# reglab/aquaculture

Measured on AMD Instinct MI355X. Metric: 640px tiles/sec (whole node) YOLOv5m bf16, higher is better.
Workload: dtype bf16

## Files before the change

aquaculture_amd/csrc/detect_nms.hip:

```cpp
#include "aq_common.h"

namespace {

constexpr float kMaxWH = 7680.0f;
constexpr int kMaxNms = 30000;
constexpr int kNmsThreads = 1024;
constexpr int kSortLds = 4096;

struct DecodeParams {
    const float* head[3];
    int head_ld;
    int B, nc, na, no;
    int ny[3], nx[3];
    int off[4];
    float stride[3];
    float anchor[3][8][2];
    float* pred;
    float conf_thres;
    int32_t* cand;
    float* cand_rows;
    int32_t* cand_count;
    int cap;
    int lmask, base, pred_rows;
    float scale, flip_w;
// ... 82 lines not shown
                if (p.cand_rows)
                    decode_row<AUG>(p, src[k], lvl[k], a[k], x[k], y[k], obj[k], p.cand_rows + ((long long)b * p.cap + pos) * p.no);
            }
        }
    }
}

struct NmsParams {
    const float* rows;
    int rows_per_tile;
    int B, N, nc, no;
    float conf_thres, iou_thres;
    int max_det;
    const int32_t* cand;
    const int32_t* cand_count;
    int cap;
    unsigned long long* keys;
    float4* sbox;
    unsigned long long* mask;
    int npow2;
    aq_det* dets;
    int32_t* counts;
    unsigned long long* dbg;
    float class_step;
    unsigned long long cls_lo, cls_hi;
};

constexpr int kFast = 2048;
constexpr int kFastBig = 4096;
constexpr int kFastRowsLimit = 40000;
__host__ __device__ constexpr int nms_fast(int N) { return N > kFastRowsLimit ? kFastBig : kFast; }
constexpr int kIdxBits = 17;
constexpr int nms_fast_lds(int kf) { return kf * 8 + kf * 16 + kf * 4 + kf * 2; }
constexpr int nms_mask_lds(int kf) { return kf == kFast ? 64 * 1024 : 32 * 1024; }
constexpr int kSlowLds = kSortLds * 8 + kMaxNms + 16;
constexpr int nms_lds(int kf) { return nms_fast_lds(kf) + nms_mask_lds(kf) > kSlowLds ? nms_fast_lds(kf) + nms_mask_lds(kf) : kSlowLds; }
static_assert(nms_lds(kFastBig) <= 160 * 1024, "LDS");

__device__ __forceinline__ bool candidate_row(const float* row, int nc, float thr, float4& box, float& conf, int& cls,
                                              unsigned long long cls_lo = ~0ULL, unsigned long long cls_hi = ~0ULL) {
    const float obj = row[4];
    if (!(obj > thr)) return false;
    float best = row[5] * obj;
    int bj = 0;
    for (int c = 1; c < nc; ++c) {
        const float v = row[5 + c] * obj;
        if (v > best) { best = v; bj = c; }
    }
    if (!(best > thr)) return false;
// ... 43 lines not shown
    if (!(inter > 0.0f)) return false;
    const float jarea = (bj.z - bj.x) * (bj.w - bj.y);
    const float uni = iarea + jarea - inter;
    const float q = inter * __builtin_amdgcn_rcpf(uni);
    if (q > thr_hi) return true;
    if (q < thr_lo) return false;
    return inter / uni > thr;
}

__device__ __forceinline__ unsigned long long readlane64(unsigned long long v, int lane) {
    const unsigned lo = (unsigned)__builtin_amdgcn_readlane((int)(unsigned)(v & 0xffffffffull), lane);
    const unsigned hi = (unsigned)__builtin_amdgcn_readlane((int)(unsigned)(v >> 32), lane);
    return ((unsigned long long)hi << 32) | lo;
}

template <int KF>
__global__ __launch_bounds__(kNmsThreads) void nms_kernel(const NmsParams p) {
    constexpr int kFast = KF, kFastWords = KF / 64, kFastLds = nms_fast_lds(KF), kMaskLds = nms_mask_lds(KF);
    __shared__ int s_n;
    extern __shared__ __attribute__((aligned(16))) unsigned char s_raw[];
    __shared__ int s_kept;
    const int b = blockIdx.x, tid = threadIdx.x;
    auto stamp = [&](int i) { if (p.dbg && tid == 0) p.dbg[(long long)b * 8 + i] = clock64(); };
    stamp(0);
    const float* rows = p.rows + (long long)b * p.rows_per_tile * p.no;
    unsigned long long* keys = p.keys + (long long)b * p.npow2;

    if (tid == 0) s_n = 0;
    __syncthreads();
    const int n0 = p.cand ? min(p.cand_count[b], p.cap) : p.N;
    for (int t = tid; t < n0; t += kNmsThreads) {
        const int idx = p.cand ? p.cand[(long long)b * p.cap + t] : t;
        float4 box; float conf; int cls;
        if (candidate_row(rows + (long long)t * p.no, p.nc, p.conf_thres, box, conf, cls, p.cls_lo, p.cls_hi)) {
            const int pos = atomicAdd(&s_n, 1);
            keys[pos] = make_key(conf, idx, t);
        }
    }
    __syncthreads();
    stamp(1);
    int n = s_n;
    if (n == 0) {
        if (tid == 0) p.counts[b] = 0;
        return;
    }

    auto emit = [&](int slot, int k) {
        float4 box; float conf; int cls;
        candidate_row(rows + (long long)slot * p.no, p.nc, p.conf_thres, box, conf, cls, p.cls_lo, p.cls_hi);
        aq_det d; d.x1 = box.x; d.y1 = box.y; d.x2 = box.z; d.y2 = box.w; d.conf = conf; d.cls = (float)cls;
        p.dets[(long long)b * p.max_det + k] = d;
    };

    if (n <= kFast) {
        unsigned long long* kin = (unsigned long long*)s_raw;
        float4* sb = (float4*)(s_raw + kFast * 8);
        int* sslot = (int*)(s_raw + kFast * 8 + kFast * 16);
        unsigned short* skept = (unsigned short*)(s_raw + kFast * 8 + kFast * 16 + kFast * 4);
        for (int t = tid; t < n; t += kNmsThreads) kin[t] = keys[t];
        __syncthreads();
        for (int t = tid; t < n; t += kNmsThreads) {
            const unsigned long long k = kin[t];
            int r = 0;
            for (int u = 0; u < n; ++u) r += (kin[u] > k) ? 1 : 0;
            sslot[r] = key_slot(k);
            float4 box; float conf; int cls;
            candidate_row(rows + (long long)key_slot(k) * p.no, p.nc, p.conf_thres, box, conf, cls, p.cls_lo, p.cls_hi);
            const float c = (float)cls * p.class_step;
            box.x = box.x + c; box.y = box.y + c; box.z = box.z + c; box.w = box.w + c;
            sb[r] = box;
        }
        __syncthreads();
        stamp(2);
        const int nw = (n + 63) >> 6;
        const float thr_lo = p.iou_thres * (1.0f - 4e-7f), thr_hi = p.iou_thres * (1.0f + 4e-7f);
        auto matrix_and_scan = [&](unsigned long long* mask) __attribute__((always_inline)) {
            int total_items = 0;
            for (int bi = 0; bi < nw; ++bi) total_items += 64 * (nw - bi);
            for (int item = tid; item < total_items; item += kNmsThreads) {
                int bi = 0, rem = item;
                while (rem >= 64 * (nw - bi)) { rem -= 64 * (nw - bi); ++bi; }
                const int wpr = nw - bi;
                const int i = 64 * bi + rem / wpr, w = bi + rem % wpr;
                if (i >= n) continue;
                const float4 bi4 = sb[i];
                const float iarea = (bi4.z - bi4.x) * (bi4.w - bi4.y);
                const int j0 = w << 6;
                const int jbeg = max(j0, i + 1), jend = min(j0 + 64, n);
                unsigned long long bits = 0ull;
#pragma unroll 4
                for (int j = jbeg; j < jend; ++j)
                    if (iou_gt_fast(bi4, iarea, sb[j], p.iou_thres, thr_lo, thr_hi)) bits |= 1ull << (j - j0);
                mask[(long long)i * nw + w] = bits;
            }
            __syncthreads();
            stamp(3);
            if (tid < 64) {
                unsigned long long removed = 0ull;
                int kept = 0;
                bool done = false;
                for (int w = 0; w < nw && !done; ++w) {
                    const int i_l = 64 * w + tid;
                    const unsigned long long diag = i_l < n ? mask[(long long)i_l * nw + w] : 0ull;
                    const int left = n - 64 * w;
                    const unsigned long long valid = left >= 64 ? ~0ull : ((1ull << left) - 1ull);
                    unsigned long long alive = valid & ~readlane64(removed, w);
                    unsigned long long keptmask = 0ull;
                    while (alive != 0ull) {
                        const int bit = __builtin_ctzll(alive);
                        keptmask |= 1ull << bit;
                        alive &= ~(1ull << bit);
                        alive &= ~readlane64(diag, bit);
                        if (kept + __builtin_popcountll(keptmask) >= p.max_det) { done = true; break; }
                    }
                    if ((keptmask >> tid) & 1ull)
                        skept[kept + __builtin_popcountll(keptmask & ((1ull << tid) - 1ull))] = (unsigned short)(64 * w + tid);
                    kept += __builtin_popcountll(keptmask);
                    unsigned long long km = keptmask, acc = 0ull;
                    const bool mine = tid > w && tid < nw;
                    while (km != 0ull) {
                        int bits4[4];
#pragma unroll
                        for (int u = 0; u < 4; ++u) {
                            bits4[u] = km != 0ull ? __builtin_ctzll(km) : -1;
                            km &= km - 1ull;
                        }
                        unsigned long long r4[4];
#pragma unroll
                        for (int u = 0; u < 4; ++u) r4[u] = (mine && bits4[u] >= 0) ? mask[(long long)(64 * w + bits4[u]) * nw + tid] : 0ull;
                        acc |= (r4[0] | r4[1]) | (r4[2] | r4[3]);
                    }
                    removed |= acc;
                }
                if (tid == 0) { p.counts[b] = kept; s_kept = kept; }
            }
        };
        if ((size_t)n * nw * 8 <= kMaskLds) matrix_and_scan((unsigned long long*)(s_raw + kFastLds));
        else matrix_and_scan(p.mask + (long long)b * kFast * kFastWords);
        __syncthreads();
        stamp(4);
        for (int k = tid; k < s_kept; k += kNmsThreads) emit(sslot[skept[k]], k);
        __syncthreads();
        stamp(5);
        return;
    }

    unsigned long long* s_keys = (unsigned long long*)s_raw;
    unsigned char* s_supp = s_raw + kSortLds * 8;
// ... 110 lines not shown
    return align_up((size_t)B * next_pow2(N) * sizeof(unsigned long long), 256) + align_up((size_t)B * N * sizeof(float4), 256) +
           align_up((size_t)B * nms_fast(N) * (nms_fast(N) / 64) * sizeof(unsigned long long), 256);
}

extern "C" int aq_nms(const float* rows_dev, int rows_per_tile, int B, int N, int nc, float conf_thres, float iou_thres,
                      int max_det, const int32_t* cand_dev, const int32_t* cand_count_dev, int cand_cap,
                      void* scratch_dev, aq_det* dets_dev, int32_t* counts_dev, void* stream) {
    return aq_nms_opts(rows_dev, rows_per_tile, B, N, nc, conf_thres, iou_thres, max_det, cand_dev, cand_count_dev, cand_cap, scratch_dev, dets_dev,
                       counts_dev, 0, ~0ULL, ~0ULL, stream);
}

extern "C" int aq_nms_opts(const float* rows_dev, int rows_per_tile, int B, int N, int nc, float conf_thres, float iou_thres,
                           int max_det, const int32_t* cand_dev, const int32_t* cand_count_dev, int cand_cap,
                           void* scratch_dev, aq_det* dets_dev, int32_t* counts_dev, int agnostic, unsigned long long classes_lo,
                           unsigned long long classes_hi, void* stream) {
    AQ_REQUIRE(nc <= 128, "nms: the class filter covers 128 classes (nc = %d)", nc);
    AQ_REQUIRE(rows_dev && scratch_dev && dets_dev && counts_dev, "nms: null pointer");
    AQ_REQUIRE(B > 0 && N > 0 && nc >= 1 && max_det > 0, "nms: bad shape B=%d N=%d nc=%d max_det=%d", B, N, nc, max_det);
    AQ_REQUIRE(N < (1 << kIdxBits), "nms: at most %d candidates per tile are supported (got %d)", (1 << kIdxBits) - 1, N);
    AQ_REQUIRE(!cand_dev || (cand_count_dev && cand_cap > 0 && cand_cap <= N && rows_per_tile == cand_cap),
               "nms: a compact candidate list needs a counter, 0 < cap <= N and rows_per_tile == cap");
    AQ_REQUIRE(cand_dev || rows_per_tile == N, "nms: without a candidate list the rows are the full pred (rows_per_tile == N)");
    NmsParams p;
    p.rows = rows_dev; p.rows_per_tile = rows_per_tile; p.B = B; p.N = N; p.nc = nc; p.no = nc + 5;
    p.conf_thres = conf_thres; p.iou_thres = iou_thres; p.max_det = max_det;
    p.cand = cand_dev; p.cand_count = cand_count_dev; p.cap = cand_cap;
    p.class_step = agnostic ? 0.0f : kMaxWH; p.cls_lo = classes_lo; p.cls_hi = classes_hi;
    p.npow2 = next_pow2(N);
    char* s = (char*)scratch_dev;
    p.keys = (unsigned long long*)s;
    s += align_up((size_t)B * p.npow2 * sizeof(unsigned long long), 256);
    p.sbox = (float4*)s;
    s += align_up((size_t)B * N * sizeof(float4), 256);
    p.mask = (unsigned long long*)s;
    p.dets = dets_dev; p.counts = counts_dev;
    p.dbg = aq_stamp_target((size_t)B * 64);
    const bool big = nms_fast(N) == kFastBig;
    auto fn = big ? nms_kernel<kFastBig> : nms_kernel<kFast>;
    const int lds = nms_lds(big ? kFastBig : kFast);
    AQ_CHECK_HIP(aq_kernel_lds((const void*)fn, lds));
    hipLaunchKernelGGL(fn, dim3(B), dim3(kNmsThreads), lds, (hipStream_t)stream, p);
// ... 4 lines not shown
```

aquaculture_amd/csrc/engine.cpp:

```cpp
#include "aq_common.h"
#include <unistd.h>
#include <string>

#include <cstdarg>
#include <cstdio>
#include <cstdlib>
#include <cstring>
#include <string>
#include <atomic>
#include <dlfcn.h>
#include <vector>

namespace {
thread_local char g_err[512] = "";
}

void aq_set_error(const char* fmt, ...) {
    va_list ap;
    va_start(ap, fmt);
    vsnprintf(g_err, sizeof(g_err), fmt, ap);
    va_end(ap);
}

extern "C" const char* aq_last_error(void) { return g_err; }
// ... 134 lines not shown
    struct Tuned { int B = 0, H = 0, W = 0; std::vector<int> cfg; };
    std::vector<Tuned> tuned;
    int tuned_cur = -1;
    bool tuning = false;
    void* zero_page = nullptr;
    int lay_B = 0, lay_H = 0, lay_W = 0;
    bool lay_aug = false;
    int run_H = 0, run_W = 0;
    std::vector<TensorPlace> place;
    size_t off_pred = 0, off_cand = 0, off_cand_rows = 0, off_cand_count = 0, off_cand_wide = 0, off_nms = 0, off_taps = 0, total_bytes = 0;
    int N = 0;
    aq_augment_pass aug[3] = {};
    std::vector<int> aug_family[3], aug_cfg[3];
    void* last_ws = nullptr;
    const uint8_t* last_tiles = nullptr;
    float* calib_amax = nullptr;
    std::vector<int> last_family, last_cfg;
    bool prof = false;
    int ring = 0;
    long long prof_calls = 0;
    std::vector<hipEvent_t> ev;
};

namespace {

void set_dims(aq_engine* e, int H, int W) {
    for (size_t t = 0; t < e->tensors.size(); ++t) {
        e->place[t].h = H / e->tensors[t].down;
        e->place[t].w = W / e->tensors[t].down;
    }
// ... 396 lines not shown
                float anchors[8 * 2];
                for (int a = 0; a < e->desc.na; ++a) {
                    anchors[2 * a] = e->desc.anchors_px[op.level][a][0];
                    anchors[2 * a + 1] = e->desc.anchors_px[op.level][a][1];
                }
                note_launch(e, oi, AQ_FAM_HEAD_DECODE);
                if (ar) {
                    rc = aq_head_decode_aug(tptr(e, ws, tiles, op.src.tensor), e->tensors[op.src.tensor].channels, op.src.ch_off, op.src.channels,
                                            e->packed[oi].w_head, B, pl.h, pl.w, aug_base + off, e->desc.stride[op.level], anchors, e->desc.nc, e->desc.na,
                                            conf, aug_scale, aug_flip_w, cand, cand_rows, wide, kCountStride, e->N, stream);
                    break;
                }
                rc = aq_head_decode(tptr(e, ws, tiles, op.src.tensor), e->tensors[op.src.tensor].channels, op.src.ch_off, op.src.channels,
                                    e->packed[oi].w_head, B, pl.h, pl.w, off, e->desc.stride[op.level], anchors, e->desc.nc, e->desc.na, conf,
                                    cand, cand_rows, wide, kCountStride, e->N, stream);
                if (!rc && ++heads_done == 3) rc = aq_head_counts_gather(wide, kCountStride, cand_count, B, stream);
                break;
            }
            rc = run_conv(e, oi, ws, tiles, B, stream);
            if (!rc && e->calib_amax && e->tensors[op.dst.tensor].dtype == AQ_T_ACT && prec == AQ_BF16 && op.dst.channels % 8 == 0) {
                const TensorPlace& pdc = e->place[op.dst.tensor];
                rc = aq_absmax_bf16(tptr(e, ws, tiles, op.dst.tensor), e->tensors[op.dst.tensor].channels, op.dst.ch_off, op.dst.channels,
                                    (long long)B * pdc.h * pdc.w, e->calib_amax + oi, stream);
            }
            break;
        case AQ_OP_STEM:
            note_launch(e, oi, AQ_FAM_STEM);
            if (stemdown) break;
            if (scaled) {
                rc = aq_stem_conv_scaled(tiles, ar->H0, ar->W0, ar->ytab, ar->xtab, ar->ps->h, ar->ps->w, tptr(e, ws, tiles, op.dst.tensor),
                                         e->tensors[op.dst.tensor].channels, op.dst.ch_off, op.dst.channels, e->packed[oi].w, e->packed[oi].bias,
// ... 38 lines not shown
        case AQ_OP_SPPF_POOL: {
            const TensorPlace& pl = e->place[op.src.tensor];
            rc = aq_sppf_pool(tptr(e, ws, tiles, op.src.tensor), e->tensors[op.src.tensor].channels, op.src.ch_off,
                              op.src.channels, B, pl.h, pl.w, prec, stream);
            break;
        }
        case AQ_OP_UPSAMPLE2X: {
            const TensorPlace& pl = e->place[op.src.tensor];
            rc = aq_upsample2x(tptr(e, ws, tiles, op.src.tensor), e->tensors[op.src.tensor].channels, op.src.ch_off,
                               tptr(e, ws, tiles, op.dst.tensor), e->tensors[op.dst.tensor].channels, op.dst.ch_off,
                               op.src.channels, B, pl.h, pl.w, prec, stream);
            break;
        }
        case AQ_OP_DECODE: {
            if (fuse_heads) break;
            const float* heads[3];
            for (int l = 0; l < 3; ++l) heads[l] = (const float*)tptr(e, ws, tiles, e->desc.head_tensor[l]);
            float anchors[3 * 8 * 2];
            for (int l = 0; l < 3; ++l)
                for (int a = 0; a < e->desc.na; ++a) {
                    anchors[(l * e->desc.na + a) * 2] = e->desc.anchors_px[l][a][0];
                    anchors[(l * e->desc.na + a) * 2 + 1] = e->desc.anchors_px[l][a][1];
                }
            const bool want_nms = dets != nullptr;
            if (ar) {
                rc = aq_detect_decode_aug(heads, e->tensors[e->desc.head_tensor[0]].channels, B, H, W, e->desc.nc, e->desc.na, anchors,
                                          e->desc.stride, ar->ps->level_mask, aug_base, e->N, aug_scale, aug_flip_w, want_nms ? nullptr : pred,
                                          conf, want_nms ? cand : nullptr, want_nms ? cand_rows : nullptr, want_nms ? cand_count : nullptr,
                                          e->N, stream);
                break;
            }
            rc = aq_detect_decode(heads, e->tensors[e->desc.head_tensor[0]].channels, B, H, W, e->desc.nc, e->desc.na,
                                  anchors, e->desc.stride, want_nms ? nullptr : pred, conf, want_nms ? cand : nullptr,
                                  want_nms ? cand_rows : nullptr, want_nms ? cand_count : nullptr, e->N, stream);
            break;
        }
        case AQ_OP_NMS:
            if (dets && !ar)
                rc = aq_nms_opts(cand_rows, e->N, B, e->N, e->desc.nc, conf, iou, max_det, cand, cand_count, e->N,
                                 (char*)ws + e->off_nms, dets, counts, e->nms_agnostic, e->nms_cls_lo, e->nms_cls_hi, stream);
            break;
        default:
            aq_set_error("unknown op kind %d", op.kind);
            rc = AQ_ERR_INVALID;
        }
        if (mark) g_roctx.pop();
        if (rc) return rc;
    }
    if (ev) {
        AQ_CHECK_HIP(hipEventRecord(ev[n_ops], stream));
        e->prof_calls++;
    }
    return AQ_OK;
}

// ... 28 lines not shown
    if (dets) {
        AQ_CHECK_HIP(hipMemsetAsync(fuse ? wide : cand_count, 0, sizeof(int32_t) * B * (fuse ? kCountStride : 1), stream));
    }
    float* pred = pred_out ? pred_out : (float*)((char*)ws + e->off_pred);
    for (int i = 0; i < 3 && !rc; ++i) {
        const aq_augment_pass& ps = e->aug[i];
        const AugRun ar{i, &ps, H, W, ytab[i], xtab[i]};
        set_dims(e, ps.hp, ps.wp);
        if (e->last_family.size() == e->ops.size()) { e->last_family.assign(e->ops.size(), AQ_FAM_NONE); e->last_cfg.assign(e->ops.size(), -1); }
        rc = run_plan(e, tiles, B, ps.hp, ps.wp, ws, ws_bytes, pred, dets, counts, conf, iou, max_det, stream, 0, -1, &ar);
        e->aug_family[i] = e->last_family;
        e->aug_cfg[i] = e->last_cfg;
    }
    set_dims(e, H, W);
    if (rc || !dets) return rc;
    if (fuse) {
        rc = aq_head_counts_gather(wide, kCountStride, cand_count, B, stream);
        if (rc) return rc;
    }
    return aq_nms_opts((float*)((char*)ws + e->off_cand_rows), e->N, B, e->N, e->desc.nc, conf, iou, max_det, (int32_t*)((char*)ws + e->off_cand),
                       cand_count, e->N, (char*)ws + e->off_nms, dets, counts, e->nms_agnostic, e->nms_cls_lo, e->nms_cls_hi, stream);
}

}

extern "C" int aq_pack_conv_weights(const float* w, int cout, int k, int cin, int precision, void* packed_dev,
                                    size_t* bytes, void* stream) {
    AQ_REQUIRE(w && bytes, "pack: null pointer");
    AQ_REQUIRE(cout > 0 && k > 0 && cin > 0 && (cin * aq_elem_bytes(precision)) % 16 == 0,
               "pack: cin=%d must make whole 16-byte groups", cin);
    std::vector<unsigned char> host;
    int kg, kgp, g, rows;
    pack_host(w, cout, k, cin, precision, host, &kg, &kgp, &g, &rows);
    *bytes = host.size();
    if (packed_dev) {
        AQ_CHECK_HIP(hipMemcpyAsync(packed_dev, host.data(), host.size(), hipMemcpyHostToDevice, (hipStream_t)stream));
// ... 101 lines not shown
    if (x3) compute_desc.precision = AQ_FP32;
    d = &compute_desc;
    e->desc = *d;
    e->tensors.assign(d->tensors, d->tensors + d->n_tensors);
    e->ops.assign(d->ops, d->ops + d->n_ops);
    e->desc.tensors = e->tensors.data();
    e->desc.ops = e->ops.data();
    e->packed.resize(e->ops.size());
    e->conv_cfg.assign(e->ops.size(), -1);
    const int eb = aq_elem_bytes(d->precision);
    auto fail = [&](int rc) { aq_engine_destroy(e); return rc; };
    if (hipMalloc(&e->zero_page, 4096) != hipSuccess || hipMemset(e->zero_page, 0, 4096) != hipSuccess) {
        aq_set_error("engine_create: zero page allocation failed");
        return fail(AQ_ERR_NOMEM);
    }
    const char* use_tail = getenv("AQ_C3TAIL");
    for (size_t oi = 0; d->precision == AQ_BF16 && !(use_tail && *use_tail == '0') && oi + 1 < e->ops.size(); ++oi) {
        const aq_op_desc& b = e->ops[oi];
        const aq_op_desc& c = e->ops[oi + 1];
        if (b.kind != AQ_OP_BOTTLENECK || c.kind != AQ_OP_CONV || !b.weight || !b.bias || !c.weight || !c.bias) continue;
        if (b.src.channels != 48 || b.dst.channels != 48 || b.k != 3 || b.dst.tensor < 0 || b.dst.tensor >= d->n_tensors || b.dst.ch_off != 0 ||
            e->tensors[b.dst.tensor].channels != 96 || b.src.tensor == b.dst.tensor)
            continue;
        if (c.k != 1 || c.stride != 1 || c.act != 1 || c.res.tensor >= 0 || c.level >= 0 || c.src.tensor != b.dst.tensor || c.src.ch_off != 0 ||
            c.src.channels != 96 || c.dst.channels != 96 || c.dst.tensor < 0 || c.dst.tensor >= d->n_tensors || c.dst.tensor == c.src.tensor ||
            c.dst.tensor == b.src.tensor || c.dst.ch_off % 8 || e->tensors[c.dst.tensor].channels % 8 || e->tensors[c.dst.tensor].dtype != AQ_T_ACT)
            continue;
        bool read_later = false;
        for (size_t oj = oi + 2; oj < e->ops.size(); ++oj)
            for (const aq_slice* s : {&e->ops[oj].src, &e->ops[oj].res})
// ... 353 lines not shown

extern "C" int aq_engine_tensor_ptr(aq_engine* e, int tensor, void** ptr, int* channels, int* h, int* w, int* elem_bytes) {
    AQ_REQUIRE(e && ptr && tensor >= 0 && tensor < (int)e->tensors.size(), "tensor_ptr: bad tensor id %d", tensor);
    AQ_REQUIRE(e->last_ws, "tensor_ptr: no call has run yet");
    *ptr = tptr(e, e->last_ws, e->last_tiles, tensor);
    if (channels) *channels = e->tensors[tensor].channels;
    if (h) *h = e->place[tensor].h;
    if (w) *w = e->place[tensor].w;
    if (elem_bytes) *elem_bytes = e->place[tensor].elem;
    return AQ_OK;
}

extern "C" int aq_engine_candidates(aq_engine* e, void** cand, void** rows, void** counts, int* cap) {
    AQ_REQUIRE(e && cand && rows && counts && cap, "candidates: null pointer");
    AQ_REQUIRE(e->last_ws, "candidates: no call has run yet");
    *cand = (char*)e->last_ws + e->off_cand;
    *rows = (char*)e->last_ws + e->off_cand_rows;
    *counts = (char*)e->last_ws + e->off_cand_count;
    *cap = e->N;
    return AQ_OK;
}

extern "C" int aq_engine_num_ops(aq_engine* e) { return e ? (int)e->ops.size() : 0; }

extern "C" int aq_engine_set_nms_options(aq_engine* e, int agnostic, unsigned long long classes_lo, unsigned long long classes_hi) {
    AQ_REQUIRE(e, "set_nms_options: null engine");
    e->nms_agnostic = agnostic != 0; e->nms_cls_lo = classes_lo; e->nms_cls_hi = classes_hi;
    return AQ_OK;
}

// ... 168 lines not shown
```

aquaculture_amd/engine.py:

```python
from __future__ import annotations

import ctypes as C
import os
import re
from typing import Dict, List, Optional, Sequence, Tuple

import numpy as np
import torch

from . import spec as _spec
from .checkpoint import Checkpoint, pack_plan_weights

AQ_BF16, AQ_FP32, AQ_BF16_W8, AQ_F16X3 = 0, 1, 2, 3
PRECISIONS = {"bf16": AQ_BF16, "fp32": AQ_FP32, "fp8w": AQ_BF16, "f16x3": AQ_F16X3}
"""Compute precision of the single-op helpers.  fp8w = fp8 (OCP e4m3fn) weights with per-output-channel power-of-two scales, bf16
activations (quant.py): values bf16 holds exactly, so every bf16 kernel runs them as they are."""
ENGINE_PRECISIONS = {"bf16": AQ_BF16, "fp32": AQ_FP32, "fp8w": AQ_BF16_W8, "f16x3": AQ_F16X3, "fp8": AQ_BF16}
"""aq_model_desc.precision.  AQ_BF16_W8 computes as AQ_BF16; kernels with an fp8-weight stream (the planar 3x3) load the e4m3 codes."""
_DTYPE_CODE = {"act": 0, "f32": 1, "u8": 2}

LIB_PATH = os.path.join(os.path.dirname(os.path.abspath(__file__)), "csrc", "libaqengine.so")


class aq_tensor_desc(C.Structure):
# ... 17 lines not shown
                ("head_tensor", C.c_int32 * 3), ("input_tensor", C.c_int32),
                ("n_tensors", C.c_int32), ("n_ops", C.c_int32),
                ("tensors", C.POINTER(aq_tensor_desc)), ("ops", C.POINTER(aq_op_desc))]


class aq_det(C.Structure):
    _fields_ = [("x1", C.c_float), ("y1", C.c_float), ("x2", C.c_float), ("y2", C.c_float),
                ("conf", C.c_float), ("cls", C.c_float)]


EXPORTS = (
    "aq_last_error", "aq_version", "aq_engine_create", "aq_engine_destroy", "aq_engine_workspace_bytes", "aq_size_guard",
    "aq_engine_infer", "aq_engine_run_ops", "aq_engine_candidates", "aq_engine_forward_raw", "aq_engine_tensor_ptr", "aq_engine_profile",
    "aq_engine_op_times", "aq_engine_num_ops", "aq_engine_set_conv_config", "aq_engine_autotune", "aq_engine_set_tuned_table",
    "aq_engine_get_conv_config", "aq_conv_num_configs", "aq_debug_conv_stamp", "aq_debug_mfma_peak",
    "aq_conv_config_tiles", "aq_pack_conv_weights", "aq_pack_conv_weights_x3", "aq_conv2d", "aq_pack_stem_weights", "aq_stem_conv", "aq_pack_bottleneck_weights", "aq_bottleneck", "aq_bottleneck_asm_form", "aq_bottleneck_c3tail_supported", "aq_pack_bottleneck_c3tail_weights", "aq_bottleneck_c3tail", "aq_pack_downblock_weights", "aq_downblock", "aq_stemdown_supported", "aq_stemdown", "aq_conv1x1_direct_supported", "aq_pack_conv1x1_direct", "aq_conv1x1_direct", "aq_conv1x1_asm_supported", "aq_pack_conv1x1_asm", "aq_conv1x1_asm", "aq_nms_opts", "aq_engine_set_nms_options",
    "aq_conv3x3s2_direct_supported", "aq_pack_conv3x3s2_direct", "aq_conv3x3s2_direct",
    "aq_conv3x3_pl_supported", "aq_conv3x3_pl_asm_family", "aq_pack_conv3x3_pl", "aq_conv3x3_pl", "aq_conv3x3_pl_s2_supported", "aq_pack_conv3x3_pl_s2", "aq_conv3x3_pl_s2", "aq_jpeg_scratch_bytes", "aq_jpeg_idct_rgb", "aq_jpeg_idct_rgb_checked", "aq_f32_to_e4m3", "aq_conv1x1_direct_f8out", "aq_absmax_bf16", "aq_engine_calibrate_amax", "aq_engine_set_fp8_scales", "aq_engine_last_launch", "aq_conv3x3_pl_f8_supported", "aq_pack_conv3x3_pl_f8", "aq_conv3x3_pl_f8", "aq_conv3x3_pl_w8_supported", "aq_pack_conv3x3_pl_w8", "aq_conv3x3_pl_w8", "aq_head_decode_supported", "aq_pack_head_weights", "aq_head_decode", "aq_head_counts_gather", "aq_preprocess_s2d", "aq_sppf_pool",
    "aq_upsample2x", "aq_letterbox_u8", "aq_letterbox_tiles_u8", "aq_format_label_rows", "aq_detect_decode", "aq_nms_scratch_bytes", "aq_nms", "aq_jpeg_huffman_decode", "aq_write_label_files",
    "aq_crop_jpeg_coefs", "aq_crop_jpeg_bytes", "aq_write_crop_files",
    "aq_annotate_u8", "aq_image_jpeg_coefs", "aq_image_jpeg_bytes", "aq_write_image_files",
    "aq_blank_stats_scratch_bytes", "aq_blank_stats_u8",
    "aq_blank_geom_scratch_bytes", "aq_blank_components_u8", "aq_blank_ring_edges_u8",
    "aq_facility_scratch_bytes", "aq_facility_dbscan_f64",
    "aq_land_scratch_bytes", "aq_land_filter_f64",
    "aq_eval_scratch_bytes", "aq_eval_member_conf_f64", "aq_box_match_f64",
    "aq_eval_subsets_scratch_bytes", "aq_eval_member_conf_subsets_f64", "aq_box_match_subsets_scratch_bytes", "aq_box_match_subsets_f64",
    "aq_model_error_match_f64", "aq_model_error_moments_f64",
    "aq_tonnage_simulate_f64", "aq_tonnage_reduce_f64", "aq_tonnage_ndtri_f64", "aq_tonnage_uniform_f64",
    "aq_depth_ranges_f64", "aq_depth_stats_f64",
    "aq_dedup_fill_u32", "aq_dedup_sets_u32", "aq_dedup_select_f64",
# ... 93 lines not shown
                              i32, i32, i32, i32, i32, i32, i32, i32, i32, vp, vp]
    lib.aq_pack_stem_weights.argtypes = [C.POINTER(f32), i32, i32, vp, C.POINTER(sz), vp]
    lib.aq_stem_conv.argtypes = [vp, vp, i32, i32, i32, vp, vp, i32, i32, i32, i32, i32, vp]
    lib.aq_pack_bottleneck_weights.argtypes = [C.POINTER(f32), C.POINTER(f32), i32, vp, C.POINTER(sz), vp]
    lib.aq_bottleneck.argtypes = [vp, i32, i32, vp, i32, i32, i32, vp, vp, i32, i32, i32, i32, vp]
    lib.aq_bottleneck_asm_form.argtypes = [i32] * 6
    lib.aq_bottleneck_c3tail_supported.argtypes = [i32, i32, i32, i32, i32, i32]
    lib.aq_pack_bottleneck_c3tail_weights.argtypes = [C.POINTER(f32), C.POINTER(f32), C.POINTER(f32), vp, C.POINTER(sz), vp]
    lib.aq_bottleneck_c3tail.argtypes = [vp, i32, i32, vp, i32, i32, vp, i32, i32, vp, vp, i32, i32, i32, i32, vp]
    lib.aq_pack_downblock_weights.argtypes = [C.POINTER(f32), C.POINTER(f32), vp, C.POINTER(sz), vp]
    lib.aq_downblock.argtypes = [vp, i32, i32, vp, i32, i32, vp, vp, i32, i32, i32, vp]
    lib.aq_conv1x1_direct_supported.argtypes = [i32, i32]
    lib.aq_pack_conv1x1_direct.argtypes = [C.POINTER(f32), i32, i32, vp, C.POINTER(sz), vp]
    lib.aq_conv1x1_direct.argtypes = [vp, i32, i32, vp, i32, i32, i32, i32, vp, vp, C.c_longlong, i32, vp]
    lib.aq_nms_opts.argtypes = [vp, i32, i32, i32, i32, f32, f32, i32, vp, vp, i32, vp, vp, vp, i32, C.c_ulonglong, C.c_ulonglong, vp]
    lib.aq_engine_set_nms_options.argtypes = [vp, i32, C.c_ulonglong, C.c_ulonglong]
    lib.aq_conv1x1_asm_supported.argtypes = [i32, i32]
    lib.aq_pack_conv1x1_asm.argtypes = [C.POINTER(f32), i32, i32, vp, C.POINTER(sz), vp]
    lib.aq_conv1x1_asm.argtypes = [vp, i32, i32, vp, i32, i32, i32, i32, vp, vp, C.c_longlong, i32, vp]
    lib.aq_conv3x3s2_direct_supported.argtypes = [i32, i32]
    lib.aq_pack_conv3x3s2_direct.argtypes = [C.POINTER(f32), i32, i32, vp, C.POINTER(sz), vp]
    lib.aq_conv3x3s2_direct.argtypes = [vp, i32, i32, vp, i32, i32, i32, i32, vp, vp, i32, i32, i32, i32, vp]
    lib.aq_conv3x3_pl_supported.argtypes = [i32, i32]
    lib.aq_conv3x3_pl_asm_family.argtypes = [i32]
    lib.aq_pack_conv3x3_pl.argtypes = [C.POINTER(f32), i32, i32, vp, C.POINTER(sz), vp]
    lib.aq_conv3x3_pl.argtypes = [vp, C.c_longlong, C.c_longlong, i32, vp, i32, i32, i32, vp, i32, i32, vp, vp, i32, i32, i32, i32, vp]
    lib.aq_conv3x3_pl_w8.argtypes = lib.aq_conv3x3_pl.argtypes
    lib.aq_pack_conv3x3_pl_w8.argtypes = [C.POINTER(C.c_float), C.POINTER(C.c_float), i32, i32, vp, C.POINTER(C.c_size_t), vp, vp]
    lib.aq_conv3x3_pl_w8_supported.argtypes = [i32] * 5
    lib.aq_jpeg_scratch_bytes.argtypes = [i32, i32, i32]
# ... 380 lines not shown
    lib = load_library()
    if pred.dtype != torch.float32 or pred.dim() != 3 or not pred.is_cuda or not pred.is_contiguous():
        raise ValueError("pred must be a contiguous CUDA float32 tensor [B, N, 5+nc]")
    B, N, no = pred.shape
    if no != nc + 5:
        raise ValueError(f"pred last dim {no} != nc + 5 = {nc + 5}")
    scratch = torch.empty(lib.aq_nms_scratch_bytes(B, N), dtype=torch.uint8, device=pred.device)
    dets = torch.empty((B, max_det, 6), dtype=torch.float32, device=pred.device)
    counts = torch.empty((B,), dtype=torch.int32, device=pred.device)
    lo, hi = class_mask(classes, nc)
    _check(lib.aq_nms_opts(pred.data_ptr(), N, B, N, nc, conf_thres, iou_thres, max_det, None, None, 0,
                           scratch.data_ptr(), dets.data_ptr(), counts.data_ptr(), int(bool(agnostic)), lo, hi, _stream_ptr()))
    return dets, counts


_zero_pages: Dict[int, torch.Tensor] = {}


def _zero_page(device) -> torch.Tensor:
    key = device.index or 0
    if key not in _zero_pages:
        _zero_pages[key] = torch.zeros(4096, dtype=torch.uint8, device=device)
    return _zero_pages[key]


def pack_conv_weights(w_oihw: torch.Tensor, precision: str, device) -> torch.Tensor:
    lib = load_library()
    prec = PRECISIONS[precision]
    w = np.ascontiguousarray(w_oihw.permute(0, 2, 3, 1).float().cpu().numpy())
    cout, k, _, cin = w.shape
# ... 1540 lines not shown
```

include/aq_engine.h:

```cpp
#ifndef AQ_ENGINE_H
#define AQ_ENGINE_H

#include <stddef.h>
#include <stdint.h>

#ifdef __cplusplus
extern "C" {
#endif

typedef enum aq_status {
    AQ_OK = 0,
    AQ_ERR_INVALID = -1,
    AQ_ERR_HIP = -2,
    AQ_ERR_NOMEM = -3,
    AQ_ERR_WORKSPACE = -4
} aq_status;

typedef enum aq_precision {
    AQ_BF16 = 0,
    AQ_FP32 = 1,
    AQ_BF16_W8 = 2,
    AQ_F16X3 = 3
} aq_precision;

// ... 215 lines not shown
                   int32_t* cand_dev, float* cand_rows_dev, int32_t* cand_count_dev, int count_stride, int cand_cap, void* stream);
int aq_head_counts_gather(const int32_t* wide_dev, int count_stride, int32_t* compact_dev, int B, void* stream);

int aq_detect_decode(const float* const head_dev[3], int head_ld, int B, int H, int W, int nc, int na,
                     const float* anchors_px , const float* stride ,
                     float* pred_dev, float conf_thres, int32_t* cand_dev, float* cand_rows_dev,
                     int32_t* cand_count_dev, int cand_cap, void* stream);
size_t aq_nms_scratch_bytes(int B, int N);
int aq_nms(const float* rows_dev, int rows_per_tile, int B, int N, int nc, float conf_thres, float iou_thres,
           int max_det, const int32_t* cand_dev, const int32_t* cand_count_dev, int cand_cap,
           void* scratch_dev, aq_det* dets_dev, int32_t* counts_dev, void* stream);
int aq_nms_opts(const float* rows_dev, int rows_per_tile, int B, int N, int nc, float conf_thres, float iou_thres,
                int max_det, const int32_t* cand_dev, const int32_t* cand_count_dev, int cand_cap,
                void* scratch_dev, aq_det* dets_dev, int32_t* counts_dev, int agnostic, unsigned long long classes_lo,
                unsigned long long classes_hi, void* stream);
int aq_engine_set_nms_options(aq_engine* e, int agnostic, unsigned long long classes_lo, unsigned long long classes_hi);

typedef struct aq_augment_pass {
    float scale;
    int32_t flip;
    int32_t h, w;
    int32_t hp, wp;
    int32_t rows;
    int32_t keep_first, keep_count;
    int32_t out_first;
    int32_t level_mask;
} aq_augment_pass;
int aq_augment_geometry(int H, int W, int na, aq_augment_pass passes_out[3], int* n_aug);
typedef struct aq_tap { int32_t i0, i1; float l0, l1; } aq_tap;
int aq_augment_taps(int in, int out, int flip, aq_tap* taps_host);
// ... 129 lines not shown
```

Baseline: 17210.

## Split NMS into per-class segments and read strided candidate counters directly

When NMS is class-aware, candidates are bucketed by class into contiguous segments. Each class then gets its own triangular IoU mask and greedy scan, run in parallel across waves, instead of one n-by-n matrix scanned by a single wave. Kept boxes are compacted back into score order with a prefix scan. Separately, the NMS kernel now reads the wide per-tile counters through a stride, which removes the counts-gather launch on the default path. The cost is extra sorting and class-rank work, more LDS bookkeeping, and a fallback whenever box coordinates exceed the segment bound.

```diff
diff --git a/aquaculture_amd/csrc/detect_nms.hip b/aquaculture_amd/csrc/detect_nms.hip
--- a/aquaculture_amd/csrc/detect_nms.hip
+++ b/aquaculture_amd/csrc/detect_nms.hip
@@ -120,7 +120,9 @@
     int max_det;
     const int32_t* cand;
     const int32_t* cand_count;
+    int count_stride;
     int cap;
+    int segments;
     unsigned long long* keys;
     float4* sbox;
     unsigned long long* mask;
@@ -139,6 +141,8 @@
 constexpr int kIdxBits = 17;
 constexpr int nms_fast_lds(int kf) { return kf * 8 + kf * 16 + kf * 4 + kf * 2; }
 constexpr int nms_mask_lds(int kf) { return kf == kFast ? 64 * 1024 : 32 * 1024; }
+constexpr int kSegTab = 4096;
+constexpr float kSegCoord = 3712.0f;
 constexpr int kSlowLds = kSortLds * 8 + kMaxNms + 16;
 constexpr int nms_lds(int kf) { return nms_fast_lds(kf) + nms_mask_lds(kf) > kSlowLds ? nms_fast_lds(kf) + nms_mask_lds(kf) : kSlowLds; }
 static_assert(nms_lds(kFastBig) <= 160 * 1024, "LDS");
@@ -212,10 +216,63 @@
     return ((unsigned long long)hi << 32) | lo;
 }
 
+__device__ __forceinline__ void matrix_word(const float4* sb, int n, int nw, int i, int w, float thr, float thr_lo, float thr_hi,
+                                            unsigned long long* mask) {
+    const float4 bi4 = sb[i];
+    const float iarea = (bi4.z - bi4.x) * (bi4.w - bi4.y);
+    const int j0 = w << 6;
+    const int jbeg = max(j0, i + 1), jend = min(j0 + 64, n);
+    unsigned long long bits = 0ull;
+#pragma unroll 4
+    for (int j = jbeg; j < jend; ++j)
+        if (iou_gt_fast(bi4, iarea, sb[j], thr, thr_lo, thr_hi)) bits |= 1ull << (j - j0);
+    mask[(long long)i * nw + w] = bits;
+}
+
+template <class Kept>
+__device__ __forceinline__ int greedy_scan(const unsigned long long* mask, int n, int nw, int lane, int max_det, Kept&& on_kept) {
+    unsigned long long removed = 0ull;
+    int kept = 0;
+    bool done = false;
+    for (int w = 0; w < nw && !done; ++w) {
+        const int i_l = 64 * w + lane;
+        const unsigned long long diag = i_l < n ? mask[(long long)i_l * nw + w] : 0ull;
+        const int left = n - 64 * w;
+        const unsigned long long valid = left >= 64 ? ~0ull : ((1ull << left) - 1ull);
+        unsigned long long alive = valid & ~readlane64(removed, w);
+        unsigned long long keptmask = 0ull;
+        while (alive != 0ull) {
+            const int bit = __builtin_ctzll(alive);
+            keptmask |= 1ull << bit;
+            alive &= ~(1ull << bit);
+            alive &= ~readlane64(diag, bit);
+            if (kept + __builtin_popcountll(keptmask) >= max_det) { done = true; break; }
+        }
+        on_kept(kept, keptmask, w);
+        kept += __builtin_popcountll(keptmask);
+        unsigned long long km = keptmask, acc = 0ull;
+        const bool mine = lane > w && lane < nw;
+        while (km != 0ull) {
+            int bits4[4];
+#pragma unroll
+            for (int u = 0; u < 4; ++u) {
+                bits4[u] = km != 0ull ? __builtin_ctzll(km) : -1;
+                km &= km - 1ull;
+            }
+            unsigned long long r4[4];
+#pragma unroll
+            for (int u = 0; u < 4; ++u) r4[u] = (mine && bits4[u] >= 0) ? mask[(long long)(64 * w + bits4[u]) * nw + lane] : 0ull;
+            acc |= (r4[0] | r4[1]) | (r4[2] | r4[3]);
+        }
+        removed |= acc;
+    }
+    return kept;
+}
+
 template <int KF>
 __global__ __launch_bounds__(kNmsThreads) void nms_kernel(const NmsParams p) {
     constexpr int kFast = KF, kFastWords = KF / 64, kFastLds = nms_fast_lds(KF), kMaskLds = nms_mask_lds(KF);
-    __shared__ int s_n;
+    __shared__ int s_n, s_bad, s_nseg, s_mwords;
     extern __shared__ __attribute__((aligned(16))) unsigned char s_raw[];
     __shared__ int s_kept;
     const int b = blockIdx.x, tid = threadIdx.x;
@@ -224,15 +281,30 @@
     const float* rows = p.rows + (long long)b * p.rows_per_tile * p.no;
     unsigned long long* keys = p.keys + (long long)b * p.npow2;
 
-    if (tid == 0) s_n = 0;
+    const bool try_seg = p.segments != 0 && p.class_step != 0.0f;
+    unsigned char* scls = s_raw + kFast * 8 + kFast * 16 + kFast * 4;
+    int* hist = (int*)(s_raw + kFastLds);
+    int* cbase = hist + 128;
+    int* seg_pos = hist + 256;
+    int* seg_n = hist + 384;
+    int* seg_moff = hist + 512;
+    int* seg_item = hist + 640;
+    static_assert((640 + 129) * 4 <= kSegTab && kSegTab < kMaskLds, "segment tables");
+    if (tid == 0) { s_n = 0; s_bad = 0; s_nseg = 0; }
+    if (try_seg && tid < 128) hist[tid] = 0;
     __syncthreads();
-    const int n0 = p.cand ? min(p.cand_count[b], p.cap) : p.N;
+    const int n0 = p.cand ? min(p.cand_count[(long long)b * p.count_stride], p.cap) : p.N;
     for (int t = tid; t < n0; t += kNmsThreads) {
         const int idx = p.cand ? p.cand[(long long)b * p.cap + t] : t;
         float4 box; float conf; int cls;
         if (candidate_row(rows + (long long)t * p.no, p.nc, p.conf_thres, box, conf, cls, p.cls_lo, p.cls_hi)) {
             const int pos = atomicAdd(&s_n, 1);
             keys[pos] = make_key(conf, idx, t);
+            if (try_seg) {
+                if (pos < kFast) scls[pos] = (unsigned char)cls;
+                atomicAdd(&hist[cls], 1);
+                if (!(fabsf(box.x) <= kSegCoord && fabsf(box.y) <= kSegCoord && fabsf(box.z) <= kSegCoord && fabsf(box.w) <= kSegCoord)) s_bad = 1;
+            }
         }
     }
     __syncthreads();
@@ -255,8 +327,119 @@
         float4* sb = (float4*)(s_raw + kFast * 8);
         int* sslot = (int*)(s_raw + kFast * 8 + kFast * 16);
         unsigned short* skept = (unsigned short*)(s_raw + kFast * 8 + kFast * 16 + kFast * 4);
+        if (try_seg && !s_bad && tid <= p.nc) {
+            int words = 0, segs = 0, moff = 0, items = 0;
+            for (int u = 0; u < p.nc; ++u) {
+                const int wu = u < tid ? (hist[u] + 63) >> 6 : 0;
+                words += wu; segs += wu ? 1 : 0; moff += 64 * wu * wu; items += 32 * wu * (wu + 1);
+            }
+            if (tid < p.nc && hist[tid] > 0) {
+                cbase[tid] = 64 * words;
+                seg_pos[segs] = 64 * words; seg_n[segs] = hist[tid]; seg_moff[segs] = moff; seg_item[segs] = items;
+            }
+            if (tid == p.nc && 64 * words <= kFast && segs > 1) { s_nseg = segs; s_mwords = moff; seg_item[segs] = items; }
+        }
         for (int t = tid; t < n; t += kNmsThreads) kin[t] = keys[t];
         __syncthreads();
+        const float thr_lo = p.iou_thres * (1.0f - 4e-7f), thr_hi = p.iou_thres * (1.0f + 4e-7f);
+        if (s_nseg > 0) {
+            const int nseg = s_nseg;
+            if (p.dbg && tid == 0) p.dbg[(long long)b * 8 + 6] = (unsigned long long)nseg;
+            unsigned char* rcls = scls + kFast;
+            int* rslot = (int*)(s_raw + kFastLds + kSegTab);
+            static_assert(kSegTab + kFast * 4 <= kMaskLds, "slots by rank");
+            for (int t = tid; t < n; t += kNmsThreads) {
+                const unsigned long long k = kin[t];
+                int r = 0;
+                for (int u = 0; u < n; ++u) r += (kin[u] > k) ? 1 : 0;
+                rcls[r] = scls[t];
+                rslot[r] = key_slot(k);
+            }
+            __syncthreads();
+            for (int r = tid; r < n; r += kNmsThreads) {
+                const int mycls = rcls[r];
+                const unsigned long long pat = 0x0101010101010101ull * (unsigned long long)mycls, lo7 = 0x7f7f7f7f7f7f7f7full;
+                int rc = 0;
+                for (int u = 0; u <= r >> 3; ++u) {
+                    unsigned long long x = ((const unsigned long long*)rcls)[u] ^ pat;
+                    if (u == r >> 3) x |= ~0ull << (8 * (r & 7));
+                    rc += __builtin_popcountll(~(((x & lo7) + lo7) | x) & ~lo7);
+                }
+                const int q = cbase[mycls] + rc;
+                const int slot = rslot[r];
+                sslot[q] = slot | (r << kIdxBits);
+                float4 box; float conf; int cls;
+                candidate_row(rows + (long long)slot * p.no, p.nc, p.conf_thres, box, conf, cls, p.cls_lo, p.cls_hi);
+                const float c = (float)cls * p.class_step;
+                box.x = box.x + c; box.y = box.y + c; box.z = box.z + c; box.w = box.w + c;
+                sb[q] = box;
+            }
+            __syncthreads();
+            stamp(2);
+            int* sout = (int*)s_raw;
+            int* wtot = sout + kFast;
+            constexpr int kPer = kFast / kNmsThreads;
+#pragma unroll
+            for (int j = 0; j < kPer; ++j) sout[tid * kPer + j] = 0;
+            auto seg_matrix_and_scan = [&](unsigned long long* mask) __attribute__((always_inline)) {
+                const int total_items = seg_item[nseg];
+                int s = 0;
+                for (int item = tid; item < total_items; item += kNmsThreads) {
+                    while (item >= seg_item[s + 1]) ++s;
+                    const int ns = seg_n[s], nws = (ns + 63) >> 6;
+                    int bi = 0, rem = item - seg_item[s];
+                    while (rem >= 64 * (nws - bi)) { rem -= 64 * (nws - bi); ++bi; }
+                    const int wpr = nws - bi;
+                    const int i = 64 * bi + rem / wpr, w = bi + rem % wpr;
+                    if (i >= ns) continue;
+                    matrix_word(sb + seg_pos[s], ns, nws, i, w, p.iou_thres, thr_lo, thr_hi, mask + seg_moff[s]);
+                }
+                __syncthreads();
+                stamp(3);
+                const int lane = tid & 63;
+                for (int si = __builtin_amdgcn_readfirstlane(tid >> 6); si < nseg; si += kNmsThreads / 64) {
+                    const int ns = seg_n[si], pos = seg_pos[si];
+                    greedy_scan(mask + seg_moff[si], ns, (ns + 63) >> 6, lane, p.max_det, [&](int, unsigned long long keptmask, int w) {
+                        if ((keptmask >> lane) & 1ull) {
+                            const int v = sslot[pos + 64 * w + lane];
+                            sout[v >> kIdxBits] = (v & ((1 << kIdxBits) - 1)) + 1;
+                        }
+                    });
+                }
+            };
+            if ((size_t)s_mwords * 8 <= kMaskLds - kSegTab) seg_matrix_and_scan((unsigned long long*)(s_raw + kFastLds + kSegTab));
+            else seg_matrix_and_scan(p.mask + (long long)b * kFast * kFastWords);
+            __syncthreads();
+            stamp(4);
+            int v[kPer], cnt = 0;
+#pragma unroll
+            for (int j = 0; j < kPer; ++j) { v[j] = sout[tid * kPer + j]; cnt += v[j] ? 1 : 0; }
+            const int lane = tid & 63, wave = tid >> 6;
+            int incl = cnt;
+#pragma unroll
+            for (int d = 1; d < 64; d <<= 1) {
+                const int o = __shfl_up(incl, d);
+                if (lane >= d) incl += o;
+            }
+            if (lane == 63) wtot[wave] = incl;
+            __syncthreads();
+            int k = incl - cnt, total = 0;
+            for (int u = 0; u < kNmsThreads / 64; ++u) {
+                const int wt = wtot[u];
+                k += u < wave ? wt : 0;
+                total += wt;
+            }
+#pragma unroll
+            for (int j = 0; j < kPer; ++j)
+                if (v[j]) {
+                    if (k < p.max_det) emit(v[j] - 1, k);
+                    ++k;
+                }
+            if (tid == 0) p.counts[b] = min(total, p.max_det);
+            __syncthreads();
+            stamp(5);
+            return;
+        }
         for (int t = tid; t < n; t += kNmsThreads) {
             const unsigned long long k = kin[t];
             int r = 0;
@@ -271,7 +454,6 @@
         __syncthreads();
         stamp(2);
         const int nw = (n + 63) >> 6;
-        const float thr_lo = p.iou_thres * (1.0f - 4e-7f), thr_hi = p.iou_thres * (1.0f + 4e-7f);
         auto matrix_and_scan = [&](unsigned long long* mask) __attribute__((always_inline)) {
             int total_items = 0;
             for (int bi = 0; bi < nw; ++bi) total_items += 64 * (nw - bi);
@@ -281,55 +463,15 @@
                 const int wpr = nw - bi;
                 const int i = 64 * bi + rem / wpr, w = bi + rem % wpr;
                 if (i >= n) continue;
-                const float4 bi4 = sb[i];
-                const float iarea = (bi4.z - bi4.x) * (bi4.w - bi4.y);
-                const int j0 = w << 6;
-                const int jbeg = max(j0, i + 1), jend = min(j0 + 64, n);
-                unsigned long long bits = 0ull;
-#pragma unroll 4
-                for (int j = jbeg; j < jend; ++j)
-                    if (iou_gt_fast(bi4, iarea, sb[j], p.iou_thres, thr_lo, thr_hi)) bits |= 1ull << (j - j0);
-                mask[(long long)i * nw + w] = bits;
+                matrix_word(sb, n, nw, i, w, p.iou_thres, thr_lo, thr_hi, mask);
             }
             __syncthreads();
             stamp(3);
             if (tid < 64) {
-                unsigned long long removed = 0ull;
-                int kept = 0;
-                bool done = false;
-                for (int w = 0; w < nw && !done; ++w) {
-                    const int i_l = 64 * w + tid;
-                    const unsigned long long diag = i_l < n ? mask[(long long)i_l * nw + w] : 0ull;
-                    const int left = n - 64 * w;
-                    const unsigned long long valid = left >= 64 ? ~0ull : ((1ull << left) - 1ull);
-                    unsigned long long alive = valid & ~readlane64(removed, w);
-                    unsigned long long keptmask = 0ull;
-                    while (alive != 0ull) {
-                        const int bit = __builtin_ctzll(alive);
-                        keptmask |= 1ull << bit;
-                        alive &= ~(1ull << bit);
-                        alive &= ~readlane64(diag, bit);
-                        if (kept + __builtin_popcountll(keptmask) >= p.max_det) { done = true; break; }
-                    }
+                const int kept = greedy_scan(mask, n, nw, tid, p.max_det, [&](int kept_before, unsigned long long keptmask, int w) {
                     if ((keptmask >> tid) & 1ull)
-                        skept[kept + __builtin_popcountll(keptmask & ((1ull << tid) - 1ull))] = (unsigned short)(64 * w + tid);
-                    kept += __builtin_popcountll(keptmask);
-                    unsigned long long km = keptmask, acc = 0ull;
-                    const bool mine = tid > w && tid < nw;
-                    while (km != 0ull) {
-                        int bits4[4];
-#pragma unroll
-                        for (int u = 0; u < 4; ++u) {
-                            bits4[u] = km != 0ull ? __builtin_ctzll(km) : -1;
-                            km &= km - 1ull;
-                        }
-                        unsigned long long r4[4];
-#pragma unroll
-                        for (int u = 0; u < 4; ++u) r4[u] = (mine && bits4[u] >= 0) ? mask[(long long)(64 * w + bits4[u]) * nw + tid] : 0ull;
-                        acc |= (r4[0] | r4[1]) | (r4[2] | r4[3]);
-                    }
-                    removed |= acc;
-                }
+                        skept[kept_before + __builtin_popcountll(keptmask & ((1ull << tid) - 1ull))] = (unsigned short)(64 * w + tid);
+                });
                 if (tid == 0) { p.counts[b] = kept; s_kept = kept; }
             }
         };
@@ -470,6 +612,15 @@
                            int max_det, const int32_t* cand_dev, const int32_t* cand_count_dev, int cand_cap,
                            void* scratch_dev, aq_det* dets_dev, int32_t* counts_dev, int agnostic, unsigned long long classes_lo,
                            unsigned long long classes_hi, void* stream) {
+    return aq_nms_opts_strided(rows_dev, rows_per_tile, B, N, nc, conf_thres, iou_thres, max_det, cand_dev, cand_count_dev, 1, cand_cap, scratch_dev,
+                               dets_dev, counts_dev, agnostic, classes_lo, classes_hi, 1, stream);
+}
+
+extern "C" int aq_nms_opts_strided(const float* rows_dev, int rows_per_tile, int B, int N, int nc, float conf_thres, float iou_thres,
+                                   int max_det, const int32_t* cand_dev, const int32_t* cand_count_dev, int count_stride, int cand_cap,
+                                   void* scratch_dev, aq_det* dets_dev, int32_t* counts_dev, int agnostic, unsigned long long classes_lo,
+                                   unsigned long long classes_hi, int class_segments, void* stream) {
+    AQ_REQUIRE(count_stride >= 1, "nms: counter stride %d", count_stride);
     AQ_REQUIRE(nc <= 128, "nms: the class filter covers 128 classes (nc = %d)", nc);
     AQ_REQUIRE(rows_dev && scratch_dev && dets_dev && counts_dev, "nms: null pointer");
     AQ_REQUIRE(B > 0 && N > 0 && nc >= 1 && max_det > 0, "nms: bad shape B=%d N=%d nc=%d max_det=%d", B, N, nc, max_det);
@@ -480,7 +631,7 @@
     NmsParams p;
     p.rows = rows_dev; p.rows_per_tile = rows_per_tile; p.B = B; p.N = N; p.nc = nc; p.no = nc + 5;
     p.conf_thres = conf_thres; p.iou_thres = iou_thres; p.max_det = max_det;
-    p.cand = cand_dev; p.cand_count = cand_count_dev; p.cap = cand_cap;
+    p.cand = cand_dev; p.cand_count = cand_count_dev; p.count_stride = count_stride; p.cap = cand_cap; p.segments = class_segments;
     p.class_step = agnostic ? 0.0f : kMaxWH; p.cls_lo = classes_lo; p.cls_hi = classes_hi;
     p.npow2 = next_pow2(N);
     char* s = (char*)scratch_dev;
diff --git a/aquaculture_amd/csrc/engine.cpp b/aquaculture_amd/csrc/engine.cpp
--- a/aquaculture_amd/csrc/engine.cpp
+++ b/aquaculture_amd/csrc/engine.cpp
@@ -172,6 +172,10 @@
     std::vector<int> aug_family[3], aug_cfg[3];
     void* last_ws = nullptr;
     const uint8_t* last_tiles = nullptr;
+    bool tail = true;
+    bool counts_wide = false;
+    hipStream_t last_stream = nullptr;
+    int last_B = 0;
     float* calib_amax = nullptr;
     std::vector<int> last_family, last_cfg;
     bool prof = false;
@@ -598,7 +602,10 @@
                 rc = aq_head_decode(tptr(e, ws, tiles, op.src.tensor), e->tensors[op.src.tensor].channels, op.src.ch_off, op.src.channels,
                                     e->packed[oi].w_head, B, pl.h, pl.w, off, e->desc.stride[op.level], anchors, e->desc.nc, e->desc.na, conf,
                                     cand, cand_rows, wide, kCountStride, e->N, stream);
-                if (!rc && ++heads_done == 3) rc = aq_head_counts_gather(wide, kCountStride, cand_count, B, stream);
+                if (!rc && ++heads_done == 3) {
+                    if (e->tail) { e->counts_wide = true; e->last_stream = stream; e->last_B = B; }
+                    else rc = aq_head_counts_gather(wide, kCountStride, cand_count, B, stream);
+                }
                 break;
             }
             rc = run_conv(e, oi, ws, tiles, B, stream);
@@ -667,6 +674,7 @@
         }
         case AQ_OP_DECODE: {
             if (fuse_heads) break;
+            e->counts_wide = false;
             const float* heads[3];
             for (int l = 0; l < 3; ++l) heads[l] = (const float*)tptr(e, ws, tiles, e->desc.head_tensor[l]);
             float anchors[3 * 8 * 2];
@@ -689,9 +697,12 @@
             break;
         }
         case AQ_OP_NMS:
-            if (dets && !ar)
-                rc = aq_nms_opts(cand_rows, e->N, B, e->N, e->desc.nc, conf, iou, max_det, cand, cand_count, e->N,
-                                 (char*)ws + e->off_nms, dets, counts, e->nms_agnostic, e->nms_cls_lo, e->nms_cls_hi, stream);
+            if (dets && !ar) {
+                const bool wide_counts = fuse_heads && e->tail;
+                rc = aq_nms_opts_strided(cand_rows, e->N, B, e->N, e->desc.nc, conf, iou, max_det, cand,
+                                         wide_counts ? (const int32_t*)((char*)ws + e->off_cand_wide) : cand_count, wide_counts ? kCountStride : 1, e->N,
+                                         (char*)ws + e->off_nms, dets, counts, e->nms_agnostic, e->nms_cls_lo, e->nms_cls_hi, e->tail ? 1 : 0, stream);
+            }
             break;
         default:
             aq_set_error("unknown op kind %d", op.kind);
@@ -750,12 +761,15 @@
     }
     set_dims(e, H, W);
     if (rc || !dets) return rc;
-    if (fuse) {
+    const bool wide_counts = fuse && e->tail;
+    e->counts_wide = wide_counts; e->last_stream = stream; e->last_B = B;
+    if (fuse && !wide_counts) {
         rc = aq_head_counts_gather(wide, kCountStride, cand_count, B, stream);
         if (rc) return rc;
     }
-    return aq_nms_opts((float*)((char*)ws + e->off_cand_rows), e->N, B, e->N, e->desc.nc, conf, iou, max_det, (int32_t*)((char*)ws + e->off_cand),
-                       cand_count, e->N, (char*)ws + e->off_nms, dets, counts, e->nms_agnostic, e->nms_cls_lo, e->nms_cls_hi, stream);
+    return aq_nms_opts_strided((float*)((char*)ws + e->off_cand_rows), e->N, B, e->N, e->desc.nc, conf, iou, max_det, (int32_t*)((char*)ws + e->off_cand),
+                               wide_counts ? wide : cand_count, wide_counts ? kCountStride : 1, e->N, (char*)ws + e->off_nms, dets, counts,
+                               e->nms_agnostic, e->nms_cls_lo, e->nms_cls_hi, e->tail ? 1 : 0, stream);
 }
 
 }
@@ -887,6 +901,8 @@
         aq_set_error("engine_create: zero page allocation failed");
         return fail(AQ_ERR_NOMEM);
     }
+    const char* use_dtail = getenv("AQ_TAIL");
+    e->tail = !(use_dtail && *use_dtail == '0');
     const char* use_tail = getenv("AQ_C3TAIL");
     for (size_t oi = 0; d->precision == AQ_BF16 && !(use_tail && *use_tail == '0') && oi + 1 < e->ops.size(); ++oi) {
         const aq_op_desc& b = e->ops[oi];
@@ -1270,6 +1286,12 @@
 extern "C" int aq_engine_candidates(aq_engine* e, void** cand, void** rows, void** counts, int* cap) {
     AQ_REQUIRE(e && cand && rows && counts && cap, "candidates: null pointer");
     AQ_REQUIRE(e->last_ws, "candidates: no call has run yet");
+    if (e->counts_wide) {
+        const int rc = aq_head_counts_gather((const int32_t*)((char*)e->last_ws + e->off_cand_wide), kCountStride,
+                                             (int32_t*)((char*)e->last_ws + e->off_cand_count), e->last_B, e->last_stream);
+        if (rc) return rc;
+        e->counts_wide = false;
+    }
     *cand = (char*)e->last_ws + e->off_cand;
     *rows = (char*)e->last_ws + e->off_cand_rows;
     *counts = (char*)e->last_ws + e->off_cand_count;
diff --git a/aquaculture_amd/engine.py b/aquaculture_amd/engine.py
--- a/aquaculture_amd/engine.py
+++ b/aquaculture_amd/engine.py
@@ -55,7 +55,7 @@
     "aq_engine_infer", "aq_engine_run_ops", "aq_engine_candidates", "aq_engine_forward_raw", "aq_engine_tensor_ptr", "aq_engine_profile",
     "aq_engine_op_times", "aq_engine_num_ops", "aq_engine_set_conv_config", "aq_engine_autotune", "aq_engine_set_tuned_table",
     "aq_engine_get_conv_config", "aq_conv_num_configs", "aq_debug_conv_stamp", "aq_debug_mfma_peak",
-    "aq_conv_config_tiles", "aq_pack_conv_weights", "aq_pack_conv_weights_x3", "aq_conv2d", "aq_pack_stem_weights", "aq_stem_conv", "aq_pack_bottleneck_weights", "aq_bottleneck", "aq_bottleneck_asm_form", "aq_bottleneck_c3tail_supported", "aq_pack_bottleneck_c3tail_weights", "aq_bottleneck_c3tail", "aq_pack_downblock_weights", "aq_downblock", "aq_stemdown_supported", "aq_stemdown", "aq_conv1x1_direct_supported", "aq_pack_conv1x1_direct", "aq_conv1x1_direct", "aq_conv1x1_asm_supported", "aq_pack_conv1x1_asm", "aq_conv1x1_asm", "aq_nms_opts", "aq_engine_set_nms_options",
+    "aq_conv_config_tiles", "aq_pack_conv_weights", "aq_pack_conv_weights_x3", "aq_conv2d", "aq_pack_stem_weights", "aq_stem_conv", "aq_pack_bottleneck_weights", "aq_bottleneck", "aq_bottleneck_asm_form", "aq_bottleneck_c3tail_supported", "aq_pack_bottleneck_c3tail_weights", "aq_bottleneck_c3tail", "aq_pack_downblock_weights", "aq_downblock", "aq_stemdown_supported", "aq_stemdown", "aq_conv1x1_direct_supported", "aq_pack_conv1x1_direct", "aq_conv1x1_direct", "aq_conv1x1_asm_supported", "aq_pack_conv1x1_asm", "aq_conv1x1_asm", "aq_nms_opts", "aq_nms_opts_strided", "aq_engine_set_nms_options",
     "aq_conv3x3s2_direct_supported", "aq_pack_conv3x3s2_direct", "aq_conv3x3s2_direct",
     "aq_conv3x3_pl_supported", "aq_conv3x3_pl_asm_family", "aq_pack_conv3x3_pl", "aq_conv3x3_pl", "aq_conv3x3_pl_s2_supported", "aq_pack_conv3x3_pl_s2", "aq_conv3x3_pl_s2", "aq_jpeg_scratch_bytes", "aq_jpeg_idct_rgb", "aq_jpeg_idct_rgb_checked", "aq_f32_to_e4m3", "aq_conv1x1_direct_f8out", "aq_absmax_bf16", "aq_engine_calibrate_amax", "aq_engine_set_fp8_scales", "aq_engine_last_launch", "aq_conv3x3_pl_f8_supported", "aq_pack_conv3x3_pl_f8", "aq_conv3x3_pl_f8", "aq_conv3x3_pl_w8_supported", "aq_pack_conv3x3_pl_w8", "aq_conv3x3_pl_w8", "aq_head_decode_supported", "aq_pack_head_weights", "aq_head_decode", "aq_head_counts_gather", "aq_preprocess_s2d", "aq_sppf_pool",
     "aq_upsample2x", "aq_letterbox_u8", "aq_letterbox_tiles_u8", "aq_format_label_rows", "aq_detect_decode", "aq_nms_scratch_bytes", "aq_nms", "aq_jpeg_huffman_decode", "aq_write_label_files",
@@ -179,6 +179,7 @@
     lib.aq_pack_conv1x1_direct.argtypes = [C.POINTER(f32), i32, i32, vp, C.POINTER(sz), vp]
     lib.aq_conv1x1_direct.argtypes = [vp, i32, i32, vp, i32, i32, i32, i32, vp, vp, C.c_longlong, i32, vp]
     lib.aq_nms_opts.argtypes = [vp, i32, i32, i32, i32, f32, f32, i32, vp, vp, i32, vp, vp, vp, i32, C.c_ulonglong, C.c_ulonglong, vp]
+    lib.aq_nms_opts_strided.argtypes = [vp, i32, i32, i32, i32, f32, f32, i32, vp, vp, i32, i32, vp, vp, vp, i32, C.c_ulonglong, C.c_ulonglong, i32, vp]
     lib.aq_engine_set_nms_options.argtypes = [vp, i32, C.c_ulonglong, C.c_ulonglong]
     lib.aq_conv1x1_asm_supported.argtypes = [i32, i32]
     lib.aq_pack_conv1x1_asm.argtypes = [C.POINTER(f32), i32, i32, vp, C.POINTER(sz), vp]
@@ -589,6 +590,31 @@
     return dets, counts
 
 
+def nms_candidates(rows: torch.Tensor, cand: torch.Tensor, counters: torch.Tensor, count_stride: int, N: int, nc: int, conf_thres=0.25,
+                   iou_thres=0.45, max_det=1000, agnostic: bool = False, classes: Optional[Sequence[int]] = None,
+                   class_segments: bool = True, dets: Optional[torch.Tensor] = None,
+                   counts: Optional[torch.Tensor] = None) -> Tuple[torch.Tensor, torch.Tensor]:
+    _require_gpu()
+    lib = load_library()
+    B, cap, no = rows.shape
+    if rows.dtype != torch.float32 or not rows.is_cuda or not rows.is_contiguous() or no != nc + 5:
+        raise ValueError("rows must be a contiguous CUDA float32 tensor [B, cap, 5 + nc]")
+    if cand.dtype != torch.int32 or tuple(cand.shape) != (B, cap) or not cand.is_contiguous() or counters.dtype != torch.int32:
+        raise ValueError("cand must be a contiguous int32 [B, cap] and counters int32")
+    if counters.numel() < (B - 1) * count_stride + 1:
+        raise ValueError("counters are shorter than (B - 1) * count_stride + 1")
+    scratch = torch.empty(lib.aq_nms_scratch_bytes(B, N), dtype=torch.uint8, device=rows.device)
+    if dets is None:
+        dets = torch.empty((B, max_det, 6), dtype=torch.float32, device=rows.device)
+    if counts is None:
+        counts = torch.empty((B,), dtype=torch.int32, device=rows.device)
+    lo, hi = class_mask(classes, nc)
+    _check(lib.aq_nms_opts_strided(rows.data_ptr(), cap, B, N, nc, conf_thres, iou_thres, max_det, cand.data_ptr(), counters.data_ptr(),
+                                   int(count_stride), cap, scratch.data_ptr(), dets.data_ptr(), counts.data_ptr(), int(bool(agnostic)), lo, hi,
+                                   int(bool(class_segments)), _stream_ptr()))
+    return dets, counts
+
+
 _zero_pages: Dict[int, torch.Tensor] = {}
 
 
diff --git a/include/aq_engine.h b/include/aq_engine.h
--- a/include/aq_engine.h
+++ b/include/aq_engine.h
@@ -253,6 +253,10 @@
                 int max_det, const int32_t* cand_dev, const int32_t* cand_count_dev, int cand_cap,
                 void* scratch_dev, aq_det* dets_dev, int32_t* counts_dev, int agnostic, unsigned long long classes_lo,
                 unsigned long long classes_hi, void* stream);
+int aq_nms_opts_strided(const float* rows_dev, int rows_per_tile, int B, int N, int nc, float conf_thres, float iou_thres,
+                        int max_det, const int32_t* cand_dev, const int32_t* cand_count_dev, int count_stride, int cand_cap,
+                        void* scratch_dev, aq_det* dets_dev, int32_t* counts_dev, int agnostic, unsigned long long classes_lo,
+                        unsigned long long classes_hi, int class_segments, void* stream);
 int aq_engine_set_nms_options(aq_engine* e, int agnostic, unsigned long long classes_lo, unsigned long long classes_hi);
 
 typedef struct aq_augment_pass {
```

Result: no change. 17210 (-0.0%).
